# xuhao1/TaichiSLAM

Hardware: AMD Instinct MI355X
Metric: depth-frames/s integrated (640x480->512^3 TSDF) (higher is better)
Workload: dtype f16 storage / f32 + int64 fixed-point arithmetic; 1 GPU; BASELINE configs[1]: single 640x480 u16 depth stream (sphere room r=3 m, 1 deg/frame) -> DenseTSDF 512^3 / 2 cm, recast_step 2, max_ray 5 m; one stream+submap per GPU

## Files before the change

### taichislam_amd/csrc/tsl_integrate.hip

```cpp
#include "tsl_tsdf.hpp"
#include <hip/hip_ext.h>

namespace tsl {

#ifdef TSL_TIMING
#define TSL_T0() const int _wv = (blockIdx.x * (int)blockDim.x + (int)threadIdx.x) >> 6
#define TSL_TICK(F, k) do { long long _n = wall_clock64(); if (lane_id() == 0 && _wv < 16384) (F).dbg[_wv * 16 + (k)] = _n; } while (0)
#else
#define TSL_T0() do {} while (0)
#define TSL_TICK(F, k) do {} while (0)
#endif

#define SCATTER_TILE 4096

struct RayRegs { float pf0, pf1, pf2, d0, d1, d2, P0, P1, P2, w; long long qden; int n; };

__device__ __forceinline__ uint32_t wave_min_u32(uint32_t v)
{
    for (int d = 32; d > 0; d >>= 1) { const uint32_t o = (uint32_t)__shfl_xor((int)v, d); v = o < v ? o : v; }
    return v;
}
__device__ __forceinline__ RayRegs make_ray(const uint4 rec, int n, const FrameParams& P)
{
    RayRegs R;
// ... 553 lines not shown
{
    if (all_small) {
#pragma unroll
        for (int q = 0; q < N; ++q) nv[q] = apply_update_f(old[q], from_fix32(qn[q]), from_fix32(qd[q]));
    } else {
#pragma unroll
        for (int q = 0; q < N; ++q) nv[q] = apply_update_f(old[q], from_fix(qn[q]), from_fix(qd[q]));
    }
}

__device__ __forceinline__ int uni(int v) { return __builtin_amdgcn_readfirstlane(v); }
#define IT_UNIT 0
#define IT_POOL 1
#define IT_SLAB 2
#define IT_NP   3
#define IT_TMALL 4
#define IT_FMASK 5
#define IT_OFF  6
#define IT_N    (IT_OFF + TSL_NB)
#define IT_WORDS (IT_N + TSL_NB + 2)
#define NRANGE (PLAN_NCLS * (TSL_NB + 1))

template <bool TEX, bool FASTDIV, int NT, int SPT, int WPE>
__global__ void __launch_bounds__(NT, WPE) k_integrate_batch(MapDev M, BatchDev B, int kind)
{
    constexpr int CSEGS = SPT * NT, VPT = TSL_BRK3 / NT, CH = VPT < FLUSH_CHUNK ? VPT : FLUSH_CHUNK;
    static_assert(VPT <= 16, "the written / first-touch masks hold 16 voxels per thread");
#ifdef TSL_EXP_SLOT16
    __shared__ ulonglong2 s_acc[TSL_BRK3];
#define S_NUM(i) s_acc[i].x
#define S_DEN(i) s_acc[i].y
#else
    __shared__ unsigned long long s_num[TSL_BRK3];
    __shared__ unsigned long long s_den[TSL_BRK3];
#define S_NUM(i) s_num[i]
#define S_DEN(i) s_den[i]
#endif
    __shared__ unsigned long long s_keys[CSEGS];
    __shared__ uint32_t s_win[TEX ? TSL_BRK3 : 1];
    __shared__ int s_bin[64];
    __shared__ int s_claim[2];
    __shared__ int s_uq[TSL_NB];
    __shared__ int s_cum[NRANGE + 1];
    __shared__ int s_it[3][IT_WORDS];
    uint32_t okmask = 0u;
#pragma unroll
    for (int q = 0; q < TSL_NB; ++q) if (q < B.n) {
        const FrameDev& Fq = B.f[q];
        if (Fq.counters[HDR_FAIL] == 0) okmask |= 1u << q;
        const int nact = min(Fq.counters[1], Fq.max_frame_bricks);
        for (int i = blockIdx.x * NT + threadIdx.x; i < nact; i += gridDim.x * NT) { const int b = Fq.act_b[i]; Fq.bhist[b] = 0; Fq.bcursor[b] = 0; }
    }
    if (threadIdx.x < TSL_NB) s_uq[threadIdx.x] = 0;
    if (threadIdx.x == 0) {
        int acc = 0, k = 0;
#ifdef TSL_CLASS_MAJOR
        for (int c = 0; c < PLAN_NCLS; ++c) {
            s_cum[k++] = acc; acc += min(B.f[0].counters[HDR_UNITS + c], B.f[0].unit_cap);
            for (int q = 0; q < TSL_NB; ++q) { s_cum[k++] = acc; if ((okmask >> q) & 1u) acc += min(B.f[q].counters[HDR_PARTS + c], B.f[q].part_cap); }
        }
#else
        for (int c = 0; c < PLAN_NCLS; ++c) { s_cum[k++] = acc; if (kind != 2) acc += min(B.f[0].counters[HDR_UNITS + c], B.f[0].unit_cap); }
        for (int c = 0; c < PLAN_NCLS; ++c)
            for (int q = 0; q < TSL_NB; ++q) { s_cum[k++] = acc; if (kind != 1 && ((okmask >> q) & 1u)) acc += min(B.f[q].counters[HDR_PARTS + c], B.f[q].part_cap); }
#endif
        s_cum[NRANGE] = acc;
        s_claim[0] = __hip_atomic_fetch_add(&B.f[0].counters[kind == 2 ? HDR_CLAIM2 : HDR_CLAIM], 1, __ATOMIC_RELAXED, __HIP_MEMORY_SCOPE_AGENT);
    }
    __syncthreads();
    const int total = uni(s_cum[NRANGE]);
    int* const claim = &B.f[0].counters[kind == 2 ? HDR_CLAIM2 : HDR_CLAIM];
    auto entry_of = [&](int r, int* kq) -> int4 {
        int k = 0;
#pragma unroll
        for (int j = 1; j < NRANGE; ++j) k += r >= uni(s_cum[j]) ? 1 : 0;
#ifdef TSL_CLASS_MAJOR
// ... 23 lines not shown
            int pool = e.z;
            if (fm == 0u) { fm = 1u; pool = -1; }
            it[IT_UNIT] = kq < 0 ? 1 : 0; it[IT_POOL] = pool; it[IT_SLAB] = kq < 0 ? 0 : e.w; it[IT_NP] = kq < 0 ? 1 : (e.y >> 16) & ((1 << PART_NP_BITS) - 1);
            it[IT_TMALL] = (int)tm; it[IT_FMASK] = (int)fm;
        }
    };
    const int r0 = uni(s_claim[0]);
    if (r0 >= total) return;
    { int kq, io, in; const int4 e = entry_of(r0, &kq); info_of(e, kq, &io, &in); commit(0, e, kq, io, in); }
    __syncthreads();
    auto steps_of = [&](int sl, uint32_t fm) -> int {
        int n = 0;
#pragma unroll
        for (int q = 0; q < TSL_NB; ++q) if ((fm >> q) & 1u) n += max(1, (uni(s_it[sl][IT_N + q]) + CSEGS - 1) / CSEGS);
        return n;
    };
    long long uniq = 0;
    int t = 0, slot = 0, c = 0; (void)t;
    int n_known = 0;
    bool exhausted = false;
    int f = __builtin_ctz((uint32_t)uni(s_it[0][IT_FMASK]));

    unsigned long long kk[SPT]; uint4 recs[SPT]; uint32_t wids[SPT];
#define TSL_SORT_DEAL(KIN, NSEG, FD)                                                                                    \
    {                                                                                                                   \
        int rr[SPT];                                                                                                    \
        _Pragma("unroll") for (int q = 0; q < SPT; ++q) {                                                               \
            const int i = q * NT + (int)threadIdx.x; rr[q] = -1;                                                        \
            if (i < (NSEG)) rr[q] = atomicAdd(&s_bin[63 - (int)(KIN[q] & 63ull)], 1);                                   \
        }                                                                                                               \
        __syncthreads();                                                                                                \
        if (threadIdx.x < 64) {                                                                                         \
            const int cb = s_bin[threadIdx.x]; int inc = cb;                                                            \
            for (int d = 1; d < 64; d <<= 1) { const int o = __shfl_up(inc, d); if ((int)threadIdx.x >= d) inc += o; }  \
            s_bin[threadIdx.x] = inc - cb;                                                                              \
        }                                                                                                               \
        __syncthreads();                                                                                                \
        _Pragma("unroll") for (int q = 0; q < SPT; ++q) if (rr[q] >= 0) s_keys[s_bin[63 - (int)(KIN[q] & 63ull)] + rr[q]] = KIN[q]; \
        __syncthreads();                                                                                                \
        _Pragma("unroll") for (int q = 0; q < SPT; ++q) {                                                               \
            const int i = q * NT + ((q & 1) ? NT - 1 - (int)threadIdx.x : (int)threadIdx.x);                            \
            if (i < (NSEG)) {                                                                                           \
                kk[q] = s_keys[i];                                                                                      \
                const int r = (int)((kk[q] >> (SEG_CNT_BITS + SEG_J_BITS)) & ((1u << STG_RAY_BITS) - 1));               \
                recs[q] = (FD).rayA[r];                                                                                 \
                wids[q] = TEX ? (FD).rayFirst[r] + 1u : 0u;                                                             \
            }                                                                                                           \
        }                                                                                                               \
        if (threadIdx.x < 64) s_bin[threadIdx.x] = 0;               \
    }
#define TSL_PRIME(SL, FQ)                                                                                               \
    {                                                                                                                   \
        const FrameDev& F0 = B.f[FQ];                                                                                   \
        const int off0 = uni(s_it[SL][IT_OFF + (FQ)]), nseg0 = min(uni(s_it[SL][IT_N + (FQ)]), CSEGS);                  \
        unsigned long long k0[SPT];                                                                                     \
        _Pragma("unroll") for (int q = 0; q < SPT; ++q) { const int i = q * NT + threadIdx.x; k0[q] = i < nseg0 ? F0.seg_sorted[off0 + i] : 0ull; } \
        TSL_SORT_DEAL(k0, nseg0, F0)                                                                                    \
    }

    {
#ifdef TSL_EXP_SLOT16
        for (int i = threadIdx.x; i < TSL_BRK3; i += NT) s_acc[i] = make_ulonglong2(0ull, 0ull);
#else
        ulonglong2* zn = reinterpret_cast<ulonglong2*>(s_num); ulonglong2* zd = reinterpret_cast<ulonglong2*>(s_den);
        for (int i = threadIdx.x; i < TSL_BRK3 / 2; i += NT) { zn[i] = make_ulonglong2(0ull, 0ull); zd[i] = make_ulonglong2(0ull, 0ull); }
#endif
        if (TEX) for (int i = threadIdx.x; i < TSL_BRK3; i += NT) s_win[i] = 0u;
        if (threadIdx.x < 64) s_bin[threadIdx.x] = 0;
        __syncthreads();
        TSL_PRIME(0, f)
    }
    uint32_t old[VPT];
// ... 30 lines not shown
        const bool has_next = !last_step || n_known >= 1;
        int fx = f, cx = c + 1, slotx = slot;
        if (last_chunk) {
            cx = 0;
            if (!last_frame) fx = f + 1 + __builtin_ctz(later);
            else if (has_next) { slotx = slot1; fx = __builtin_ctz((uint32_t)uni(s_it[slotx][IT_FMASK])); }
        }
        const FrameDev& Fx = B.f[fx];
        unsigned long long kn[SPT];
        const int offx = uni(s_it[slotx][IT_OFF + fx]) + cx * CSEGS;
        const int nsegn = has_next ? min(CSEGS, uni(s_it[slotx][IT_N + fx]) - cx * CSEGS) : 0;
#pragma unroll
        for (int q = 0; q < SPT; ++q) { const int i = q * NT + threadIdx.x; kn[q] = i < nsegn ? Fx.seg_sorted[offx + i] : 0ull; }
        const uint32_t* const twr = M.tw + (size_t)(p >= 0 ? p : 0) * TSL_BRK3;
        if (first_step) { have_old = false; vmask = 0u; }
        if (!TEX && unit && p >= 0 && first_step) {
#pragma unroll
            for (int q = 0; q < VPT; ++q) old[q] = twr[q * NT + threadIdx.x];
            have_old = true;
        }
#pragma unroll
        for (int q = 0; q < SPT; ++q) {
            const int i = q * NT + ((q & 1) ? NT - 1 - (int)threadIdx.x : (int)threadIdx.x);
            if (i >= nseg) continue;
            const unsigned long long key = kk[q];
            const int cnt = (int)(key & ((1u << SEG_CNT_BITS) - 1)), j0 = (int)((key >> SEG_CNT_BITS) & ((1u << SEG_J_BITS) - 1));
            const RayRegs R = make_ray(recs[q], 0, P);
            const uint32_t wid = wids[q];
#ifndef TSL_EXP_STAGGER
#define TSL_EXP_STAGGER 27
#endif
            int off = ((int)((threadIdx.x * (unsigned)TSL_EXP_STAGGER) & 63u) * cnt) >> 6;
            for (int s = 0; s < cnt; s += 2) {
                const int ja = j0 + off; off = (off + 1 == cnt) ? 0 : off + 1;
                const int jb = j0 + off; off = (off + 1 == cnt) ? 0 : off + 1;
                int la, lb; float qa, qb;
                step_eval<FASTDIV>(R, K, ja, &la, &qa);
                step_eval<FASTDIV>(R, K, jb, &lb, &qb);
                long long na = (long long)(int)qa, nb = (long long)(int)qb;
                if (__builtin_expect(__any(!(fabsf(qa) < 2147483648.0f) || !(fabsf(qb) < 2147483648.0f)), 0)) { na = __float2ll_rn(qa); nb = __float2ll_rn(qb); }
                atomicAdd(&S_NUM(la), (unsigned long long)na);
                atomicAdd(&S_DEN(la), (unsigned long long)R.qden);
                if (TEX) atomicMax(&s_win[la], wid);
                const bool vb = s + 1 < cnt;
#ifdef TSL_EXP_ADDZERO
                atomicAdd(&S_NUM(lb), (unsigned long long)(vb ? nb : 0ll));
                atomicAdd(&S_DEN(lb), (unsigned long long)(vb ? R.qden : 0ll));
// ... 93 lines not shown
        const long long _td = wall_clock64();
#endif
        {
            const long long u = wave_sum_ll(uniq);
            if (lane_id() == 0 && u) atomicAdd(&s_uq[f], (int)u);
            uniq = 0;
        }
        if (fetching) { commit(n_known == 0 ? slot1 : slot2, ne, nkq, nio, nin); ++n_known; }
#ifdef TSL_TIMING
        if (threadIdx.x == 0 && last_step) _rec[4] = wall_clock64();
        if (threadIdx.x == 0) { _ph[2] += _td - _tc; _ph[3] += wall_clock64() - _td; }
#endif
        if (!has_next && n_known == 0) break;
        __syncthreads();
        c = 0;
        if (last_frame) { ++t; slot = slot1; --n_known; f = __builtin_ctz((uint32_t)uni(s_it[slot][IT_FMASK])); }
        else f = fx;
        if (!has_next) TSL_PRIME(slot, f)
    }
#undef TSL_PRIME
#undef TSL_SORT_DEAL
    __syncthreads();
    if (threadIdx.x < TSL_NB && s_uq[threadIdx.x]) atomic_add_i64(&B.f[threadIdx.x].stats->unique, (long long)s_uq[threadIdx.x]);
}

#ifndef APPLY_SPLIT
#define APPLY_SPLIT 8
#endif
#ifndef APPLY_ROUND
#define APPLY_ROUND 2
#endif
template <bool TEX>
__global__ void __launch_bounds__(256) k_apply_slab(MapDev M, BatchDev B)
{
    __shared__ int s_uq[TSL_NB];
    constexpr int VP = TSL_BRK3 / APPLY_SPLIT / 256;
    uint32_t okmask = 0u;
#pragma unroll
    for (int q = 0; q < TSL_NB; ++q) if (q < B.n && B.f[q].counters[HDR_FAIL] == 0) okmask |= 1u << q;
    const int nheavy = min(B.f[0].counters[HDR_HEAVY], B.f[0].max_frame_bricks);
    const ulonglong2* const slab = reinterpret_cast<const ulonglong2*>(B.f[0].acc);
    if (threadIdx.x < TSL_NB) s_uq[threadIdx.x] = 0;
    __syncthreads();
    for (int item = blockIdx.x; item < nheavy * APPLY_SPLIT; item += gridDim.x) {
        const int4 e = B.f[0].heavy_tab[item / APPLY_SPLIT];
        const int b = e.x, p = e.y;
// ... 83 lines not shown
int launch_segments(tsl_tsdf* m, const BatchDev& B, const FrameParams* hp, int total, hipStream_t st)
{
    const FrameParams& P = hp[0];
    if (P.variant != 2) return TSL_OK;
    const int iblocks = (int)(((int64_t)total * P.split + 255) / 256);
    prof_begin(m, TSL_K_SEGMENTS, st);
    if (P.group) hipLaunchKernelGGL(k_segments<true>, dim3(iblocks, B.n), dim3(256), 0, st, m->M, B);
    else hipLaunchKernelGGL(k_segments<false>, dim3(iblocks, B.n), dim3(256), 0, st, m->M, B);
    prof_end(m, st);
    int unit_max = m->unit_max <= m->unit_floor ? m->unit_max : std::max(m->unit_floor, (int)((long long)m->unit_max * B.n / TSL_NB));
    int unit_half = std::min(unit_max, m->unit_half <= 2048 ? m->unit_half : std::max(2048, (int)((long long)m->unit_half * B.n / TSL_NB)));
    if (P.seq && m->seq_impl) unit_max = unit_half = 1 << 30;
    prof_begin(m, TSL_K_BIN, st);
    hipLaunchKernelGGL(k_plan, dim3((B.f[0].max_frame_bricks + 255) / 256, B.n), dim3(256), 0, st, m->M, B, m->chunks * m->wg * m->spt, unit_max, unit_half);
    hipLaunchKernelGGL(k_scatter, dim3(256, B.n), dim3(256), 0, st, B);
    prof_end(m, st);
    return TSL_OK;
}

int launch_brick(tsl_tsdf* m, const BatchDev& B, const FrameParams& P, int kind, hipStream_t st, hipEvent_t start, hipEvent_t stop)
{
    const int bg = kind == 2 ? m->pgrid : (B.n <= 2 ? (m->bgrid + 1) / 2 : (kind == 1 ? m->ugrid : m->bgrid));
#define TSL_LAUNCH_IB(TEXV, FD) do { \
        if (m->wg == 512 && m->spt == 2 && !TEXV) hipExtLaunchKernelGGL((k_integrate_batch<false, FD, 512, 2, 4>), dim3((2 * m->ncu * bg + 99) / 100), dim3(512), 0, st, start, stop, 0, m->M, B, kind); \
        else if (m->wg == 512) hipExtLaunchKernelGGL((k_integrate_batch<TEXV, FD, 512, 4, 2>), dim3((m->ncu * bg + 99) / 100), dim3(512), 0, st, start, stop, 0, m->M, B, kind); \
        else hipExtLaunchKernelGGL((k_integrate_batch<TEXV, FD, 256, 4, (TEXV ? 1 : 2)>), dim3(((TEXV ? 1 : 2) * m->ncu * bg + 99) / 100), dim3(256), 0, st, start, stop, 0, m->M, B, kind); } while (0)
    if (P.tex) { if (P.fastdiv) TSL_LAUNCH_IB(true, true); else TSL_LAUNCH_IB(true, false); }
    else { if (P.fastdiv) TSL_LAUNCH_IB(false, true); else TSL_LAUNCH_IB(false, false); }
#undef TSL_LAUNCH_IB
    TSL_HIP(hipGetLastError());
    return TSL_OK;
}
int launch_slab_apply(tsl_tsdf* m, const BatchDev& B, const FrameParams& P)
{
    prof_begin(m, TSL_K_FINALIZE);
    if (P.tex) hipLaunchKernelGGL(k_apply_slab<true>, dim3(16 * m->ncu), dim3(256), 0, m->stream_, m->M, B);
    else hipLaunchKernelGGL(k_apply_slab<false>, dim3(16 * m->ncu), dim3(256), 0, m->stream_, m->M, B);
    prof_end(m);
    TSL_HIP(hipGetLastError());
    return TSL_OK;
}
int launch_apply_batch(tsl_tsdf* m, const BatchDev& B, const FrameParams& P, hipEvent_t start, hipEvent_t stop)
{
    const int rc = launch_brick(m, B, P, 0, m->stream_, start, stop);
    return rc ? rc : launch_slab_apply(m, B, P);
}

int launch_apply(tsl_tsdf* m, FSet& S, int total)
{
// ... 16 lines not shown
```

### taichislam_amd/csrc/tsl_tsdf.hip

```cpp
#include "tsl_tsdf.hpp"
#include <rocprim/rocprim.hpp>
#include <algorithm>
#include <cmath>
#include <cstdio>
#include <cstdlib>
#include <cstring>
#include <mutex>

namespace tsl {

static thread_local std::string g_err;
void set_error(const std::string& s) { g_err = s; }

__device__ __forceinline__ uint32_t part1by2_32(uint32_t x)
{
    x &= 0x3ffu;
    x = (x ^ (x << 16)) & 0xff0000ffu;
    x = (x ^ (x << 8)) & 0x0300f00fu;
    x = (x ^ (x << 4)) & 0x030c30c3u;
    x = (x ^ (x << 2)) & 0x09249249u;
    return x;
}
__device__ __forceinline__ uint64_t part1by2_64(uint64_t x)
{
// ... 318 lines not shown
        uint32_t* ob = reinterpret_cast<uint32_t*>(M.obs + (size_t)p * TSL_BRK3);
        uint32_t* oc = reinterpret_cast<uint32_t*>(M.occ + (size_t)p * TSL_BRK3);
        for (int l = threadIdx.x; l < TSL_BRK3; l += 256) tw[l] = 0u;
        for (int l = threadIdx.x; l < TSL_BRK3 / 4; l += 256) { ob[l] = 0u; oc[l] = 0u; }
        if (M.col) { uint2* c = reinterpret_cast<uint2*>(M.col + (size_t)p * TSL_BRK3 * 4); for (int l = threadIdx.x; l < TSL_BRK3; l += 256) c[l] = make_uint2(0u, 0u); }
        if (threadIdx.x == 0) M.table[M.owner[p]] = TSL_EMPTY;
    }
}

__global__ void __launch_bounds__(256) k_verify_div(float vs, float rvs, unsigned long long* bad)
{
    unsigned long long nbad = 0;
    for (unsigned long long i = (unsigned long long)blockIdx.x * 256 + threadIdx.x; i < (1ull << 32); i += (unsigned long long)gridDim.x * 256) {
        const float x = __uint_as_float((uint32_t)i);
        const float ax = fabsf(x);
        if (!(ax >= 7.8886090522101181e-31f) || !(ax < 2147483648.0f * vs)) continue;
        const float q = x / vs;
        const float f = div_vs(x, vs, rvs, 1);
        if (__float_as_uint(q) != __float_as_uint(f)) ++nbad;
    }
    if (nbad) atomicAdd(bad, nbad);
}

__global__ void __launch_bounds__(256) k_selftest(int which, unsigned long long* bad)
{
    unsigned long long nbad = 0;
    for (unsigned long long i = (unsigned long long)blockIdx.x * 256 + threadIdx.x; i < (1ull << 32); i += (unsigned long long)gridDim.x * 256) {
        const float x = __uint_as_float((uint32_t)i);
        if (which == 0) {
            if (!(fabsf(x) < 2147483648.0f)) continue;
            if (rnd_i(x) != rnd_i_ref(x)) ++nbad;
        } else {
            if (!(x >= 1.2621774483536189e-29f) || !(x < INFINITY)) continue;
            if (__float_as_uint(sqrt_rn_norm(x)) != __float_as_uint(sqrt_rn(x))) ++nbad;
        }
    }
    if (nbad) atomicAdd(bad, nbad);
}

int grow(void** p, size_t* have, size_t need)
{
    if (*have >= need) return TSL_OK;
    if (*p) (void)hipFree(*p);
    *p = nullptr; *have = 0;
    size_t want = need + need / 4 + 4096;
    TSL_HIP(hipMalloc(p, want));
    *have = want;
    return TSL_OK;
}
// ... 417 lines not shown
                                      (size_t)m->F.max_points, 0u, 64u, m->stream_));
    *bytes = a > b ? a : b;
    return TSL_OK;
}

static void fill_frame_params(tsl_tsdf* m, const double R[9], const double T[3])
{
    const int s = m->active;
    convert_pose(&m->baseR[(size_t)s * 9], &m->baseT[(size_t)s * 3], R, T, m->P.R, m->P.T);
    m->P.slot = map_slot(m, s);
    m->P.variant = m->variant; m->P.split = (m->variant == 2 && m->split > 8) ? 8 : m->split;
}

}

using namespace tsl;

extern "C" {

const char* tsl_version(void) { return "taichislam_hip 0.1 (gfx950)"; }
const char* tsl_last_error(void) { return g_err.c_str(); }
int tsl_selftest(int which, int64_t* mismatches)
{
    TSL_REQUIRE(mismatches && which >= 0 && which <= 2, "tsl_selftest: bad argument");
    unsigned long long* bad = nullptr;
    TSL_HIP(hipMalloc((void**)&bad, sizeof(unsigned long long)));
    TSL_HIP(hipMemset(bad, 0, sizeof(unsigned long long)));
    if (which == 2) (void)selftest_seqdiv(bad);
    else hipLaunchKernelGGL(k_selftest, dim3(8192), dim3(256), 0, 0, which, bad);
    unsigned long long h = ~0ull;
    hipError_t e = hipMemcpy(&h, bad, sizeof(h), hipMemcpyDeviceToHost);
    (void)hipFree(bad);
    TSL_HIP(e);
    *mismatches = (int64_t)h;
    return TSL_OK;
}
int tsl_device_count(int* n)
{
    int c = 0;
    hipError_t e = hipGetDeviceCount(&c);
    if (e != hipSuccess) { c = 0; }
    if (n) *n = c;
    return TSL_OK;
}

static int init_handle(tsl_tsdf* m, const tsl_tsdf_cfg* cfg, int device)
{
    m->cfg = *cfg; m->device = device; m->bytes = 0;
    (void)hipGetLastError();
    TSL_HIP(hipStreamCreateWithFlags(&m->stream_, hipStreamNonBlocking));
    m->overlap = TSL_NB; m->last_set = 0;
    for (auto& S : m->fset) { S.sort_temp = nullptr; S.header = nullptr; S.Pd = nullptr; S.stage_in = nullptr; S.stage_in_bytes = 0; S.stage_tex = nullptr; S.stage_tex_bytes = 0; S.pin = nullptr; S.pin_bytes = 0; S.pin_dev = nullptr; S.copy_in = S.copy_tex = S.copy_tex_off = 0; }
// ... 21 lines not shown
    FrameParams& P = m->P; std::memset(&P, 0, sizeof(P));
    for (int i = 0; i < 3; ++i) P.R[i * 4] = 1.0f;
    P.vs = (float)cfg->voxel_scale;
    {
        const float y0 = (float)(1.0 / (double)P.vs);
        float best = y0; double err = std::fabs(1.0 - (double)y0 * (double)P.vs);
        const float cand[2] = { std::nextafterf(y0, 0.0f), std::nextafterf(y0, INFINITY) };
        for (float c : cand) { const double e = std::fabs(1.0 - (double)c * (double)P.vs); if (e < err) { err = e; best = c; } }
        P.rvs = best; P.fastdiv = 0;
    }
    P.thr_max = (float)(cfg->max_ray_length * 1000.0); P.thr_min = (float)(cfg->min_ray_length * 1000.0);
    P.max_ray_f = (float)cfg->max_ray_length;
    P.max_steps_f = (float)(cfg->max_ray_length / cfg->voxel_scale);
    P.internal_f = (float)cfg->internal_voxels;
    P.pcl_lo = m->pcl_lo; P.pcl_ext = m->pcl_ext; P.pcl_bits = m->pcl_bits; P.pcl_blk = blk; P.seq = 0;
    P.step = cfg->recast_step; P.same_proj = cfg->color_same_proj;
    m->surf_thres = (float)(cfg->voxel_scale * 1.8);
    m->disp_floor = (float)cfg->disp_floor; m->disp_ceiling = (float)cfg->disp_ceiling;
    m->baseR.assign((size_t)m->npose * 9, 0.0); m->baseT.assign((size_t)m->npose * 3, 0.0);
    m->baseRf.assign((size_t)m->npose * 9, 0.0f); m->baseTf.assign((size_t)m->npose * 3, 0.0f);
    for (int s = 0; s < m->npose; ++s) for (int i = 0; i < 3; ++i) { m->baseR[(size_t)s * 9 + i * 4] = 1.0; m->baseRf[(size_t)s * 9 + i * 4] = 1.0f; }
    std::memset(m->gbaseR, 0, sizeof(m->gbaseR)); std::memset(m->gbaseT, 0, sizeof(m->gbaseT));
    for (int i = 0; i < 3; ++i) m->gbaseR[i * 4] = 1.0;
    m->P.group = 1; m->phases = 3; m->wg = 512; m->spt = 2; m->adaptive = 0; m->ramp_batches = 2; m->ramp_size = 4; m->bgrid = 75; m->ugrid = 75; m->pgrid = 25; m->split_launch = 0; m->chunks = 4; m->unit_max = 1024 * TSL_NB; m->unit_half = 1 << 20; m->unit_floor = 4096; m->batch_gen = 0;
    { hipDeviceProp_t pr; TSL_HIP(hipGetDeviceProperties(&pr, device)); m->ncu = pr.multiProcessorCount > 0 ? pr.multiProcessorCount : 256; }
    m->active = 0; m->variant = 2; m->split = 2; m->semantics = 0; m->seq_impl = 1; m->seq_ready = false; m->seq_bytes0 = 0; m->seq_d = nullptr; m->seq_tuple_cap = 0;
    m->prof_on = false; m->prof_open = false; m->prof_group = false; m->prof_mask = ~0u; std::memset(m->prof_ms, 0, sizeof(m->prof_ms)); std::memset(m->prof_n, 0, sizeof(m->prof_n));
    m->sort_temp = nullptr; m->sort_temp_bytes = 0;
    m->xbuf = nullptr; m->xbuf_bytes = 0; m->mesh_v = m->mesh_n = m->mesh_c = nullptr; m->mesh_count = nullptr; m->mesh_cap = 0; m->mesh_flags = nullptr;
    m->fuse_acc = nullptr; m->fuse_cnt = nullptr; m->fuse_cacc = nullptr; m->fuse_dirty = false; m->mrg_nunion = -1;
    m->esdf = nullptr; m->esdf_par = nullptr; m->esdf_ok = nullptr; m->esdf_mode = 0; m->esdf_grid = 0; m->fuse_direct = false; m->merge_exchange = 0; m->mrg_racc = m->mrg_rcnt = m->mrg_rec = nullptr; m->mrg_racc_bytes = m->mrg_rcnt_bytes = m->mrg_rec_bytes = 0; m->esdf_orphans = 0; m->esdf_last = nullptr; m->esdf_in = nullptr; m->esdf_read = nullptr; m->esdf_overlap = true; m->esdf_ctr_idx = 0; for (int k = 0; k < 2; ++k) { m->fseq_keys[k] = m->fseq_vals[k] = nullptr; m->fseq_bytes[k] = m->fseq_vbytes[k] = 0; } m->fseq_temp = nullptr; m->fseq_tbytes = 0; m->fseq_ctr = nullptr; m->esdf_gate = nullptr; m->esdf_gate_ev = nullptr; m->esdf_gate_set = false; m->esdf_gate_mask = 0; m->esdf_valid = false; m->esdf_force_full = false; m->pose_dev = nullptr;

    MapDev& M = m->M; std::memset(&M, 0, sizeof(M));
    M.N = m->N; M.Nz = m->Nz; M.nbx = m->nbx; M.nbz = m->nbz; M.nb3 = m->nb3; M.nsub = m->nsub; M.hN = m->N / 2; M.hNz = m->Nz / 2;
    int64_t want = cfg->max_bricks > 0 ? cfg->max_bricks : 32768 * (int64_t)(m->nsub > 4 ? 4 : (m->nsub > 1 ? m->nsub : 1));
    const int64_t all = (int64_t)m->nsub * m->nb3;
    if (want > all) want = all;
    M.max_bricks = (int)want;
    int rc;
    if ((rc = dev_alloc(m, (void**)&M.table, sizeof(int) * (size_t)all, 0xff))) return rc;
    if ((rc = dev_alloc(m, (void**)&M.tw, sizeof(uint32_t) * (size_t)want * TSL_BRK3, 0))) return rc;
    if ((rc = dev_alloc(m, (void**)&M.obs, (size_t)want * TSL_BRK3, 0))) return rc;
    if ((rc = dev_alloc(m, (void**)&M.occ, (size_t)want * TSL_BRK3, 0))) return rc;
    if (cfg->texture_enabled) { if ((rc = dev_alloc(m, (void**)&M.col, sizeof(uint16_t) * 4 * (size_t)want * TSL_BRK3, 0))) return rc; }
    if ((rc = dev_alloc(m, (void**)&M.owner, sizeof(int) * (size_t)want, 0))) return rc;
    if ((rc = dev_alloc(m, (void**)&M.touch, (size_t)want, 0))) return rc;
    if ((rc = dev_alloc(m, (void**)&M.pool_top, sizeof(int) * 4, 0))) return rc;
// ... 145 lines not shown
{
    TSL_HIP(hipMemcpyAsync(m->h_ints, dev, sizeof(int), hipMemcpyDeviceToHost, ms(m)));
    TSL_HIP(hipStreamSynchronize(ms(m)));
    *out = m->h_ints[0];
    return take_deferred(m);
}
static int check_dev_err(tsl_tsdf* m) { (void)ms(m); return take_dev_err(m); }
int tsl_tsdf_get_option(tsl_tsdf* m, const char* name, int* value)
{
    TSL_REQUIRE(m && name && value, "null");
    if (!std::strcmp(name, "group")) { *value = m->P.group; return TSL_OK; }
    if (!std::strcmp(name, "esdf_mode")) { *value = m->esdf_mode; return TSL_OK; }
    if (!std::strcmp(name, "fuse_window_misses")) { return read_int(m, m->M.pool_top + 2, value); }
    if (!std::strcmp(name, "esdf_orphans")) { int rc = esdf_finish(m); if (rc) return rc; *value = (int)m->esdf_orphans; return TSL_OK; }
    if (!std::strcmp(name, "semantics")) { *value = m->semantics; return TSL_OK; }
    if (!std::strcmp(name, "seq_impl")) { *value = m->seq_impl; return TSL_OK; }
    if (!std::strcmp(name, "last_heavy_bricks") || !std::strcmp(name, "last_slab_slots")) {
        TSL_REQUIRE(m->scratch_ready, "nothing integrated yet");
        int rc = tsl_tsdf_sync(m); if (rc) return rc;
        const int bi = (m->cur + TSL_NBATCH - 1) % TSL_NBATCH;
        int v[40];
        TSL_HIP(hipMemcpy(v, m->fset[bi * TSL_NB].F.counters, sizeof(v), hipMemcpyDeviceToHost));
        *value = name[5] == 'h' ? v[14] : v[13];
        return TSL_OK;
    }
    if (!std::strcmp(name, "seq_longest_run")) {
        TSL_REQUIRE(m->scratch_ready, "nothing integrated yet");
        int rc = tsl_tsdf_sync(m); if (rc) return rc;
        const int bi = (m->cur + TSL_NBATCH - 1) % TSL_NBATCH;
        long long sum = 0;
        for (int q = 0; q < m->last_batch_n; ++q) { int v[40]; TSL_HIP(hipMemcpy(v, m->fset[bi * TSL_NB + q].F.counters, sizeof(v), hipMemcpyDeviceToHost)); sum += (unsigned)v[31]; }
        *value = (int)(sum > 0x7fffffffll ? 0x7fffffffll : sum);
        return TSL_OK;
    }
    if (!std::strcmp(name, "seq_long_voxels")) {
        TSL_REQUIRE(m->scratch_ready, "nothing integrated yet");
        int rc = tsl_tsdf_sync(m); if (rc) return rc;
        const int bi = (m->cur + TSL_NBATCH - 1) % TSL_NBATCH;
        int v[40]; TSL_HIP(hipMemcpy(v, m->fset[bi * TSL_NB].F.counters, sizeof(v), hipMemcpyDeviceToHost));
        *value = v[28] + v[30];
#ifdef TSL_SEQ_DBG
        fprintf(stderr, "seq dbg (long role, last batch): evaluations %d, commits that moved T %d, commits that moved W only %d\n", v[32], v[33], v[34]);
#endif
        return TSL_OK;
    }
    if (!std::strcmp(name, "fastdiv")) { *value = m->P.fastdiv; return TSL_OK; }
// ... 387 lines not shown
                if (seq_prepare(m)) m->semantics = 0;
                return rc;
            }
        }
        return TSL_OK;
    }
    if (!std::strcmp(name, "fastdiv")) { if (value == 0) m->P.fastdiv = 0; return TSL_OK; }
    if (!std::strcmp(name, "mesh_gather")) { m->mesh_gather = value != 0; return TSL_OK; }
    if (!std::strcmp(name, "esdf_full")) { m->esdf_force_full = value != 0; return TSL_OK; }
    if (!std::strcmp(name, "esdf_mode")) { TSL_REQUIRE(value == 0 || value == 1, "esdf_mode: 0 = regional recompute (default), 1 = raise / lower wavefront with parent directions"); int rc = esdf_finish(m); if (rc) return rc; m->esdf_mode = value; m->esdf_valid = false; return TSL_OK; }
    if (!std::strcmp(name, "esdf_round_cap")) { m->esdf_round_cap = value; return TSL_OK; }
    if (!std::strcmp(name, "merge_exchange")) { TSL_REQUIRE(value == 0 || value == 1, "merge_exchange: 0 = all-reduce of the packed sums, 1 = reduce-scatter + all-gather of finalised voxels"); m->merge_exchange = value; return TSL_OK; }
    if (!std::strcmp(name, "fuse_direct")) { m->fuse_direct = value != 0; return TSL_OK; }
    if (!std::strcmp(name, "esdf_grid")) { TSL_REQUIRE(value >= 0, "esdf_grid: workgroups of a relaxation round (0 = four per CU)"); m->esdf_grid = value; return TSL_OK; }
    if (!std::strcmp(name, "esdf_overlap")) { int rc = esdf_finish(m); if (rc) return rc; m->esdf_overlap = value != 0; return TSL_OK; }
    if (!std::strcmp(name, "unit")) { TSL_REQUIRE(value >= 0 && value <= (1 << 20), "unit must be 0..2^20 segments"); int rc = tsl_tsdf_sync(m); if (rc) return rc; m->unit_max = value; return TSL_OK; }
    if (!std::strcmp(name, "unit_floor")) { TSL_REQUIRE(value >= 0 && value <= (1 << 20), "unit_floor must be 0..2^20 segments"); int rc = tsl_tsdf_sync(m); if (rc) return rc; m->unit_floor = value; return TSL_OK; }
    if (!std::strcmp(name, "unit_half")) { TSL_REQUIRE(value >= 0 && value <= (1 << 20), "unit_half must be 0..2^20 segments"); int rc = tsl_tsdf_sync(m); if (rc) return rc; m->unit_half = value; return TSL_OK; }
    if (!std::strcmp(name, "chunks")) { TSL_REQUIRE(value >= 1 && value <= 8, "chunks must be 1..8"); int rc = tsl_tsdf_sync(m); if (rc) return rc; m->chunks = value; return TSL_OK; }
    if (!std::strcmp(name, "adaptive")) { m->adaptive = value != 0; return TSL_OK; }
    if (!std::strcmp(name, "ramp_size")) { TSL_REQUIRE(value >= 1 && value <= TSL_NB, "ramp_size must be 1..8 frames"); m->ramp_size = value; return TSL_OK; }
    if (!std::strcmp(name, "ramp")) { TSL_REQUIRE(value >= 0 && value <= 16, "ramp must be 0..16 half batches"); m->ramp_batches = value; return TSL_OK; }
    if (!std::strcmp(name, "ugrid") || !std::strcmp(name, "pgrid")) { TSL_REQUIRE(value >= 5 && value <= 200, "ugrid / pgrid must be 5..200 (percent of the resident workgroup slots)"); { int rc = tsl_tsdf_sync(m); if (rc) return rc; } (name[0] == 'u' ? m->ugrid : m->pgrid) = value; return TSL_OK; }
    if (!std::strcmp(name, "split_launch")) { TSL_REQUIRE(value == 0 || value == 1, "split_launch must be 0 or 1"); { int rc = tsl_tsdf_sync(m); if (rc) return rc; } m->split_launch = value; return TSL_OK; }
    if (!std::strcmp(name, "bgrid")) { TSL_REQUIRE(value >= 10 && value <= 200, "bgrid must be 10..200 (percent of the resident workgroup slots)"); { int rc = tsl_tsdf_sync(m); if (rc) return rc; } m->bgrid = value; return TSL_OK; }
    if (!std::strcmp(name, "spt")) { TSL_REQUIRE(value == 2 || value == 4, "spt must be 2 or 4"); { int rc = tsl_tsdf_sync(m); if (rc) return rc; } m->spt = value; return TSL_OK; }
    if (!std::strcmp(name, "wg")) { TSL_REQUIRE(value == 256 || value == 512, "wg must be 256 or 512"); { int rc = tsl_tsdf_sync(m); if (rc) return rc; } m->wg = value; return TSL_OK; }
    if (!std::strcmp(name, "phases")) { int rc = tsl_tsdf_sync(m); if (rc) return rc; m->phases = value & 3; return TSL_OK; }
    if (!std::strcmp(name, "overlap")) { int rc = tsl_tsdf_sync(m); if (rc) return rc; m->overlap = value < 0 ? 0 : (value > TSL_NB ? TSL_NB : value); for (auto& H : m->batch) H.b_pending = false; return TSL_OK; }
    if (!std::strcmp(name, "split")) { TSL_REQUIRE(value >= 1 && value <= 64 && (64 % value) == 0, "split must divide 64"); m->split = value; return TSL_OK; }
    set_error("unknown option"); return TSL_ERR_ARG;
}

}
```

### taichislam_amd/csrc/tsl_tsdf.hpp

```cpp
#pragma once
#include "tsl_common.hpp"

namespace tsl {

struct FrameParams {
    float R[9], T[3];
    float fx, fy, cx, cy;
    float fxc, fyc, cxc, cyc;
    float vs;
    float rvs; int fastdiv;
    float thr_max, thr_min;
    float max_ray_f;
    float max_steps_f;
    float internal_f;
    int   pcl_lo, pcl_ext, pcl_bits;
    int   step, hh, ww, H, W;
    int   rstride;
    int   cstride;
    int   th, tw, tex, same_proj;
    int   slot;
    int   variant, split;
    int   group;
    int   seq, pcl_blk;
    int   hlog2;
// ... 35 lines not shown
#define SEG_CNT_BITS 6
#define SEG_J_BITS   12
#define SEG_RAY_BITS 24
#define SEG_SLOT_SHIFT (SEG_CNT_BITS + SEG_J_BITS + SEG_RAY_BITS)
#define SEG_MAX_CNT 63
#define STG_RAY_BITS 22
#define STG_B_SHIFT (SEG_CNT_BITS + SEG_J_BITS + STG_RAY_BITS)
#define PART_NP_BITS 12
#define SLAB_SLOT_BITS 20
#define PLAN_NCLS 4
#define HDR_FAIL 11
#define HDR_CLAIM 12
#define HDR_SLAB 13
#define HDR_HEAVY 14
#define HDR_PARTS 16
#define HDR_UNITS 20
#define HDR_CLAIM2 24
#define HDR_SEQ_TUPLES 26
#define HDR_SEQ_LONG 28
#define HDR_SEQ_XLONG 30
#define HDR_SEQ_MAXRUN 31
#define HDR_SEQ_CLAIM 35
#define HDR_SEQ_SLOTS 29

__device__ __forceinline__ void frame_fail(const MapDev& M, const FrameDev& F, int bits) { atomicOr(&F.counters[11], bits); atomicOr(M.err, bits); }

#define H_INL 13
#define H_BLOCK_SHIFT 44
#define H_EMPTY 0ull
__device__ __forceinline__ unsigned long long h_key(unsigned long long vkey, int block) { return (vkey | ((unsigned long long)block << H_BLOCK_SHIFT)) + 1ull; }
#define GROUP_BIG_CAP 16384
struct HSlot { unsigned long long key; int cnt; uint32_t pix[H_INL]; };
static_assert(sizeof(HSlot) == 64, "one slot per 64 bytes");
__device__ __forceinline__ uint32_t h_hash64(unsigned long long key, int log2n) { return (uint32_t)((key * 0x9E3779B97F4A7C15ull) >> (64 - log2n)); }

struct PixAcc { int cnt; h16 sx, sy, sz, zs, cr, cg, cb; };

__device__ __forceinline__ void acc_colour(const FrameParams& P, const FrameDev& F, uint32_t pid, PixAcc& A)
{
    const uint8_t* rgb;
    if (P.points) rgb = P.tex_input + (size_t)pid * 3;
    else {
        const int jj = (int)pid / P.ww, ii = (int)pid - jj * P.ww;
        const int pj = jj * P.step, pi = ii * P.step;
        if (P.same_proj) rgb = P.tex_input + ((size_t)pj * P.tw + pi) * 3;
        else {
// ... 118 lines not shown
    uint32_t* mesh_flags;
    float *mesh_v, *mesh_n, *mesh_c; int* mesh_count; int64_t mesh_cap; int mesh_gather;
    void *fuse_acc, *fuse_cnt, *fuse_cacc; bool fuse_dirty;
    uint8_t* mrg_mask; int *mrg_list, *mrg_count; int mrg_nunion;
    void *mrg_pacc, *mrg_pcnt; size_t mrg_pacc_bytes, mrg_pcnt_bytes;
    void *mrg_racc, *mrg_rcnt, *mrg_rec; size_t mrg_racc_bytes, mrg_rcnt_bytes, mrg_rec_bytes; int merge_exchange;
    float* esdf; uint8_t *esdf_fl, *esdf_region, *esdf_par, *esdf_ok; int esdf_mode, esdf_grid; bool fuse_direct; long long esdf_orphans; int *esdf_list, *esdf_queue, *esdf_ctr, *esdf_inq, *esdf_nbr; uint32_t* esdf_note; int esdf_qcap;
    float *esdf_exp_xyz, *esdf_exp_val; int* esdf_exp_count; int esdf_exp_n;
    bool esdf_valid, esdf_force_full; int esdf_submap; float esdf_gamma, esdf_maxd; tsl_esdf_stats esdf_stats;
    bool esdf_query_ok; int* esdf_q_ctr; int esdf_q_rounds;
    hipEvent_t esdf_gate, esdf_gate_ev; bool esdf_gate_set; unsigned esdf_gate_mask;
    hipEvent_t esdf_in, esdf_read, esdf_last;
    bool esdf_overlap; int esdf_ctr_idx;
    void *fseq_keys[2], *fseq_vals[2], *fseq_temp; size_t fseq_bytes[2], fseq_vbytes[2], fseq_tbytes; void* fseq_ctr;
    EsdfSlot esdf_slot[TSL_ESDF_SLOTS]; int esdf_tail, esdf_npend, esdf_rounds_seen, esdf_round_cap; bool esdf_short; tsl_esdf_totals_t esdf_tot;
    bool prof_on, prof_open, prof_group; unsigned prof_mask; std::vector<tsl::ProfSlot> prof; std::vector<hipEvent_t> prof_free;
    double prof_ms[TSL_K_COUNT]; int64_t prof_n[TSL_K_COUNT];
    int semantics;
    int seq_impl;
    bool seq_ready; int64_t seq_bytes0;
    tsl::SeqDev seq_h[TSL_NSETS]; tsl::SeqDev* seq_d;
    void *seqb_keys[TSL_NBATCH][2], *seqb_vals[TSL_NBATCH][2], *seqb_temp[TSL_NBATCH], *seqb_long[TSL_NBATCH], *seqb_lmask[TSL_NBATCH], *seqb_perm[TSL_NBATCH]; size_t seqb_temp_bytes; long long seq_tuple_cap;
    unsigned long long *seq_keys[2], *seq_vals[2], *seq_ctr; void* seq_temp; size_t seq_temp_bytes; long long seq_cap;
    int variant, split, phases, wg, spt, ncu, chunks, unit_max, unit_half, unit_floor, bgrid, ugrid, pgrid, split_launch, adaptive, ramp, ramp_batches, ramp_size; bool clean; uint64_t batch_gen;
    int64_t bytes;
    void* seqv_sum[TSL_NBATCH]; int* seqv_log;
    uint32_t shape_hash; int dry_launches;
};

namespace tsl {
int  grow(void** p, size_t* have, size_t need);
hipStream_t ms(tsl_tsdf* m);
int  flush_pending(tsl_tsdf* m);
void prof_begin(tsl_tsdf* m, int kid, hipStream_t st = nullptr, int count = 1);
void prof_end(tsl_tsdf* m, hipStream_t st = nullptr);
bool prof_slot(tsl_tsdf* m, int kid, int count, hipEvent_t* a, hipEvent_t* b);
void convert_pose(const double* Rb, const double* Tb, const double* R, const double* T, float* outR, float* outT);
int  dev_alloc(tsl_tsdf* m, void** p, size_t bytes, int fill);
int  check_variant2(tsl_tsdf* m);
int  launch_segments(tsl_tsdf* m, const BatchDev& B, const FrameParams* hp, int total, hipStream_t st);
int  launch_apply(tsl_tsdf* m, FSet& S, int total);
int  launch_apply_batch(tsl_tsdf* m, const BatchDev& B, const FrameParams& P, hipEvent_t start = nullptr, hipEvent_t stop = nullptr);
int  launch_brick(tsl_tsdf* m, const BatchDev& B, const FrameParams& P, int kind, hipStream_t st, hipEvent_t start, hipEvent_t stop);
int  launch_slab_apply(tsl_tsdf* m, const BatchDev& B, const FrameParams& P);
int  launch_seq_group(tsl_tsdf* m, const BatchDev& B, const FrameParams* hp, int bi, hipStream_t st);
int  launch_seq_apply(tsl_tsdf* m, const BatchDev& B, const FrameParams& P, int bi);
void seq_release(tsl_tsdf* m);
// ... 8 lines not shown
```

Measured before the change: 34530 frames/s.

## Split ray segments into pieces across idle threads in light integrate steps

When a step in the batched integrate kernel has few segments relative to the workgroup's segment capacity, each segment is dealt out in up to 2^seg_split pieces with even-length voxel counts, so more threads share the per-ray march work. This targets underutilised workgroups on light steps. The cost is extra key decoding, redundant ray-record loads per piece, and per-block counter atomics for split statistics. A selftest and a tunable knob (default max split) are added.

```diff
diff --git a/taichislam_amd/csrc/tsl_integrate.hip b/taichislam_amd/csrc/tsl_integrate.hip
--- a/taichislam_amd/csrc/tsl_integrate.hip
+++ b/taichislam_amd/csrc/tsl_integrate.hip
@@ -599,8 +599,9 @@
 #define NRANGE (PLAN_NCLS * (TSL_NB + 1))
 
 template <bool TEX, bool FASTDIV, int NT, int SPT, int WPE>
-__global__ void __launch_bounds__(NT, WPE) k_integrate_batch(MapDev M, BatchDev B, int kind)
-{
+__global__ void __launch_bounds__(NT, WPE) k_integrate_batch(MapDev M, BatchDev B, int kind_cap)
+{
+    const int kind = kind_cap & 3, split_cap = kind_cap >> 2;
     constexpr int CSEGS = SPT * NT, VPT = TSL_BRK3 / NT, CH = VPT < FLUSH_CHUNK ? VPT : FLUSH_CHUNK;
     static_assert(VPT <= 16, "the written / first-touch masks hold 16 voxels per thread");
 #ifdef TSL_EXP_SLOT16
@@ -618,6 +619,7 @@
     __shared__ int s_bin[64];
     __shared__ int s_claim[2];
     __shared__ int s_uq[TSL_NB];
+    __shared__ int s_split[SEG_SPLIT_MAX + 1];
     __shared__ int s_cum[NRANGE + 1];
     __shared__ int s_it[3][IT_WORDS];
     uint32_t okmask = 0u;
@@ -629,6 +631,7 @@
         for (int i = blockIdx.x * NT + threadIdx.x; i < nact; i += gridDim.x * NT) { const int b = Fq.act_b[i]; Fq.bhist[b] = 0; Fq.bcursor[b] = 0; }
     }
     if (threadIdx.x < TSL_NB) s_uq[threadIdx.x] = 0;
+    if (threadIdx.x <= SEG_SPLIT_MAX) s_split[threadIdx.x] = 0;
     if (threadIdx.x == 0) {
         int acc = 0, k = 0;
 #ifdef TSL_CLASS_MAJOR
@@ -698,6 +701,7 @@
     int f = __builtin_ctz((uint32_t)uni(s_it[0][IT_FMASK]));
 
     unsigned long long kk[SPT]; uint4 recs[SPT]; uint32_t wids[SPT];
+    int wsh = 0;
 #define TSL_SORT_DEAL(KIN, NSEG, FD)                                                                                    \
     {                                                                                                                   \
         int rr[SPT];                                                                                                    \
@@ -714,16 +718,20 @@
         __syncthreads();                                                                                                \
         _Pragma("unroll") for (int q = 0; q < SPT; ++q) if (rr[q] >= 0) s_keys[s_bin[63 - (int)(KIN[q] & 63ull)] + rr[q]] = KIN[q]; \
         __syncthreads();                                                                                                \
+        const int sh_ = seg_split_shift((NSEG), CSEGS, split_cap);                                                      \
         _Pragma("unroll") for (int q = 0; q < SPT; ++q) {                                                               \
             const int i = q * NT + ((q & 1) ? NT - 1 - (int)threadIdx.x : (int)threadIdx.x);                            \
-            if (i < (NSEG)) {                                                                                           \
-                kk[q] = s_keys[i];                                                                                      \
+            if (i < ((NSEG) << sh_)) {                                                                                  \
+                kk[q] = s_keys[i >> sh_];                                                                               \
+                if (sh_) kk[q] = seg_piece(kk[q], sh_, i & ((1 << sh_) - 1));        \
                 const int r = (int)((kk[q] >> (SEG_CNT_BITS + SEG_J_BITS)) & ((1u << STG_RAY_BITS) - 1));               \
                 recs[q] = (FD).rayA[r];                                                                                 \
                 wids[q] = TEX ? (FD).rayFirst[r] + 1u : 0u;                                                             \
             }                                                                                                           \
         }                                                                                                               \
         if (threadIdx.x < 64) s_bin[threadIdx.x] = 0;               \
+        if (threadIdx.x == 0 && (NSEG) > 0) atomicAdd(&s_split[sh_], 1);    \
+        wsh = sh_;                                                                                                      \
     }
 #define TSL_PRIME(SL, FQ)                                                                                               \
     {                                                                                                                   \
@@ -800,7 +808,7 @@
 #pragma unroll
         for (int q = 0; q < SPT; ++q) {
             const int i = q * NT + ((q & 1) ? NT - 1 - (int)threadIdx.x : (int)threadIdx.x);
-            if (i >= nseg) continue;
+            if (i >= (nseg << wsh)) continue;
             const unsigned long long key = kk[q];
             const int cnt = (int)(key & ((1u << SEG_CNT_BITS) - 1)), j0 = (int)((key >> SEG_CNT_BITS) & ((1u << SEG_J_BITS) - 1));
             const RayRegs R = make_ray(recs[q], 0, P);
@@ -940,6 +948,7 @@
 #undef TSL_SORT_DEAL
     __syncthreads();
     if (threadIdx.x < TSL_NB && s_uq[threadIdx.x]) atomic_add_i64(&B.f[threadIdx.x].stats->unique, (long long)s_uq[threadIdx.x]);
+    if (threadIdx.x <= SEG_SPLIT_MAX && s_split[threadIdx.x]) atomicAdd(&B.f[0].counters[HDR_SPLIT + threadIdx.x], s_split[threadIdx.x]);
 }
 
 #ifndef APPLY_SPLIT
@@ -1069,9 +1078,9 @@
 {
     const int bg = kind == 2 ? m->pgrid : (B.n <= 2 ? (m->bgrid + 1) / 2 : (kind == 1 ? m->ugrid : m->bgrid));
 #define TSL_LAUNCH_IB(TEXV, FD) do { \
-        if (m->wg == 512 && m->spt == 2 && !TEXV) hipExtLaunchKernelGGL((k_integrate_batch<false, FD, 512, 2, 4>), dim3((2 * m->ncu * bg + 99) / 100), dim3(512), 0, st, start, stop, 0, m->M, B, kind); \
-        else if (m->wg == 512) hipExtLaunchKernelGGL((k_integrate_batch<TEXV, FD, 512, 4, 2>), dim3((m->ncu * bg + 99) / 100), dim3(512), 0, st, start, stop, 0, m->M, B, kind); \
-        else hipExtLaunchKernelGGL((k_integrate_batch<TEXV, FD, 256, 4, (TEXV ? 1 : 2)>), dim3(((TEXV ? 1 : 2) * m->ncu * bg + 99) / 100), dim3(256), 0, st, start, stop, 0, m->M, B, kind); } while (0)
+        if (m->wg == 512 && m->spt == 2 && !TEXV) hipExtLaunchKernelGGL((k_integrate_batch<false, FD, 512, 2, 4>), dim3((2 * m->ncu * bg + 99) / 100), dim3(512), 0, st, start, stop, 0, m->M, B, kind | (m->seg_split << 2)); \
+        else if (m->wg == 512) hipExtLaunchKernelGGL((k_integrate_batch<TEXV, FD, 512, 4, 2>), dim3((m->ncu * bg + 99) / 100), dim3(512), 0, st, start, stop, 0, m->M, B, kind | (m->seg_split << 2)); \
+        else hipExtLaunchKernelGGL((k_integrate_batch<TEXV, FD, 256, 4, (TEXV ? 1 : 2)>), dim3(((TEXV ? 1 : 2) * m->ncu * bg + 99) / 100), dim3(256), 0, st, start, stop, 0, m->M, B, kind | (m->seg_split << 2)); } while (0)
     if (P.tex) { if (P.fastdiv) TSL_LAUNCH_IB(true, true); else TSL_LAUNCH_IB(true, false); }
     else { if (P.fastdiv) TSL_LAUNCH_IB(false, true); else TSL_LAUNCH_IB(false, false); }
 #undef TSL_LAUNCH_IB
diff --git a/taichislam_amd/csrc/tsl_tsdf.hip b/taichislam_amd/csrc/tsl_tsdf.hip
--- a/taichislam_amd/csrc/tsl_tsdf.hip
+++ b/taichislam_amd/csrc/tsl_tsdf.hip
@@ -364,9 +364,47 @@
     if (nbad) atomicAdd(bad, nbad);
 }
 
+__device__ int selftest_split_case(int i)
+{
+    if (i < 64 * 3 * 4) {
+        const int cnt = i & 63, sh = (i >> 6) & 3, jsel = i >> 8;
+        const int j0 = jsel == 0 ? 0 : (jsel == 1 ? 1 : 4032);
+        int nbad = 0;
+        for (int pat = 0; pat < 2; ++pat) {
+            const unsigned long long hi = (pat ? 0xa5c3961e5a3c69e1ull : ~0ull) << (SEG_CNT_BITS + SEG_J_BITS);
+            const unsigned long long key = hi | ((unsigned long long)j0 << SEG_CNT_BITS) | (unsigned long long)cnt;
+            const int len = ((cnt + (2 << sh) - 1) >> (sh + 1)) << 1;
+            unsigned long long seen = 0ull; bool ok = (len & 1) == 0;
+            for (int u = 0; u < (1 << sh); ++u) {
+                const unsigned long long pk = seg_piece(key, sh, u);
+                const int c = (int)(pk & 63ull), j = (int)((pk >> SEG_CNT_BITS) & 4095ull);
+                ok = ok && (pk >> (SEG_CNT_BITS + SEG_J_BITS)) == (key >> (SEG_CNT_BITS + SEG_J_BITS)) && c <= len;
+                for (int s = 0; s < c; ++s) {
+                    const int r = j + s - j0;
+                    if (r < 0 || r >= cnt || ((seen >> r) & 1ull)) ok = false; else seen |= 1ull << r;
+                }
+            }
+            ok = ok && seen == (1ull << cnt) - 1ull;
+            nbad += ok ? 0 : 1;
+        }
+        return nbad;
+    }
+    i -= 64 * 3 * 4;
+    const int nseg = i % 2049, csegs = ((i / 2049) & 1) ? 2048 : 1024, cap = i / (2049 * 2);
+    const int sh = seg_split_shift(nseg, csegs, cap);
+    if (sh < 0 || sh > cap) return 1;
+    if (nseg > csegs) return sh == 0 ? 0 : 1;
+    if ((nseg << sh) > csegs) return 1;
+    return sh == cap || (nseg << (sh + 1)) > csegs ? 0 : 1;
+}
 __global__ void __launch_bounds__(256) k_selftest(int which, unsigned long long* bad)
 {
     unsigned long long nbad = 0;
+    if (which == 3) {
+        for (int i = blockIdx.x * 256 + threadIdx.x; i < 64 * 3 * 4 + 2049 * 2 * (SEG_SPLIT_MAX + 1); i += gridDim.x * 256) nbad += selftest_split_case(i);
+        if (nbad) atomicAdd(bad, nbad);
+        return;
+    }
     for (unsigned long long i = (unsigned long long)blockIdx.x * 256 + threadIdx.x; i < (1ull << 32); i += (unsigned long long)gridDim.x * 256) {
         const float x = __uint_as_float((uint32_t)i);
         if (which == 0) {
@@ -830,12 +868,12 @@
 const char* tsl_last_error(void) { return g_err.c_str(); }
 int tsl_selftest(int which, int64_t* mismatches)
 {
-    TSL_REQUIRE(mismatches && which >= 0 && which <= 2, "tsl_selftest: bad argument");
+    TSL_REQUIRE(mismatches && which >= 0 && which <= 3, "tsl_selftest: bad argument");
     unsigned long long* bad = nullptr;
     TSL_HIP(hipMalloc((void**)&bad, sizeof(unsigned long long)));
     TSL_HIP(hipMemset(bad, 0, sizeof(unsigned long long)));
     if (which == 2) (void)selftest_seqdiv(bad);
-    else hipLaunchKernelGGL(k_selftest, dim3(8192), dim3(256), 0, 0, which, bad);
+    else hipLaunchKernelGGL(k_selftest, dim3(which == 3 ? 128 : 8192), dim3(256), 0, 0, which, bad);
     unsigned long long h = ~0ull;
     hipError_t e = hipMemcpy(&h, bad, sizeof(h), hipMemcpyDeviceToHost);
     (void)hipFree(bad);
@@ -903,7 +941,7 @@
     for (int s = 0; s < m->npose; ++s) for (int i = 0; i < 3; ++i) { m->baseR[(size_t)s * 9 + i * 4] = 1.0; m->baseRf[(size_t)s * 9 + i * 4] = 1.0f; }
     std::memset(m->gbaseR, 0, sizeof(m->gbaseR)); std::memset(m->gbaseT, 0, sizeof(m->gbaseT));
     for (int i = 0; i < 3; ++i) m->gbaseR[i * 4] = 1.0;
-    m->P.group = 1; m->phases = 3; m->wg = 512; m->spt = 2; m->adaptive = 0; m->ramp_batches = 2; m->ramp_size = 4; m->bgrid = 75; m->ugrid = 75; m->pgrid = 25; m->split_launch = 0; m->chunks = 4; m->unit_max = 1024 * TSL_NB; m->unit_half = 1 << 20; m->unit_floor = 4096; m->batch_gen = 0;
+    m->P.group = 1; m->phases = 3; m->wg = 512; m->spt = 2; m->adaptive = 0; m->ramp_batches = 2; m->ramp_size = 4; m->bgrid = 75; m->ugrid = 75; m->pgrid = 25; m->split_launch = 0; m->seg_split = SEG_SPLIT_MAX; m->chunks = 4; m->unit_max = 1024 * TSL_NB; m->unit_half = 1 << 20; m->unit_floor = 4096; m->batch_gen = 0;
     { hipDeviceProp_t pr; TSL_HIP(hipGetDeviceProperties(&pr, device)); m->ncu = pr.multiProcessorCount > 0 ? pr.multiProcessorCount : 256; }
     m->active = 0; m->variant = 2; m->split = 2; m->semantics = 0; m->seq_impl = 1; m->seq_ready = false; m->seq_bytes0 = 0; m->seq_d = nullptr; m->seq_tuple_cap = 0;
     m->prof_on = false; m->prof_open = false; m->prof_group = false; m->prof_mask = ~0u; std::memset(m->prof_ms, 0, sizeof(m->prof_ms)); std::memset(m->prof_n, 0, sizeof(m->prof_n));
@@ -1095,6 +1133,16 @@
         int v[40];
         TSL_HIP(hipMemcpy(v, m->fset[bi * TSL_NB].F.counters, sizeof(v), hipMemcpyDeviceToHost));
         *value = name[5] == 'h' ? v[14] : v[13];
+        return TSL_OK;
+    }
+    if (!std::strcmp(name, "seg_split")) { *value = m->seg_split; return TSL_OK; }
+    if (!std::strncmp(name, "last_split_steps", 16) && name[16] >= '0' && name[16] <= '0' + SEG_SPLIT_MAX && !name[17]) {
+        TSL_REQUIRE(m->scratch_ready, "nothing integrated yet");
+        int rc = tsl_tsdf_sync(m); if (rc) return rc;
+        const int bi = (m->cur + TSL_NBATCH - 1) % TSL_NBATCH;
+        int v[40];
+        TSL_HIP(hipMemcpy(v, m->fset[bi * TSL_NB].F.counters, sizeof(v), hipMemcpyDeviceToHost));
+        *value = v[HDR_SPLIT + (name[16] - '0')];
         return TSL_OK;
     }
     if (!std::strcmp(name, "seq_longest_run")) {
@@ -1528,6 +1576,7 @@
     if (!std::strcmp(name, "ramp_size")) { TSL_REQUIRE(value >= 1 && value <= TSL_NB, "ramp_size must be 1..8 frames"); m->ramp_size = value; return TSL_OK; }
     if (!std::strcmp(name, "ramp")) { TSL_REQUIRE(value >= 0 && value <= 16, "ramp must be 0..16 half batches"); m->ramp_batches = value; return TSL_OK; }
     if (!std::strcmp(name, "ugrid") || !std::strcmp(name, "pgrid")) { TSL_REQUIRE(value >= 5 && value <= 200, "ugrid / pgrid must be 5..200 (percent of the resident workgroup slots)"); { int rc = tsl_tsdf_sync(m); if (rc) return rc; } (name[0] == 'u' ? m->ugrid : m->pgrid) = value; return TSL_OK; }
+    if (!std::strcmp(name, "seg_split")) { TSL_REQUIRE(value >= 0 && value <= SEG_SPLIT_MAX, "seg_split must be 0..3 (a light step deals a segment out in up to 2^seg_split pieces)"); { int rc = tsl_tsdf_sync(m); if (rc) return rc; } m->seg_split = value; return TSL_OK; }
     if (!std::strcmp(name, "split_launch")) { TSL_REQUIRE(value == 0 || value == 1, "split_launch must be 0 or 1"); { int rc = tsl_tsdf_sync(m); if (rc) return rc; } m->split_launch = value; return TSL_OK; }
     if (!std::strcmp(name, "bgrid")) { TSL_REQUIRE(value >= 10 && value <= 200, "bgrid must be 10..200 (percent of the resident workgroup slots)"); { int rc = tsl_tsdf_sync(m); if (rc) return rc; } m->bgrid = value; return TSL_OK; }
     if (!std::strcmp(name, "spt")) { TSL_REQUIRE(value == 2 || value == 4, "spt must be 2 or 4"); { int rc = tsl_tsdf_sync(m); if (rc) return rc; } m->spt = value; return TSL_OK; }
diff --git a/taichislam_amd/csrc/tsl_tsdf.hpp b/taichislam_amd/csrc/tsl_tsdf.hpp
--- a/taichislam_amd/csrc/tsl_tsdf.hpp
+++ b/taichislam_amd/csrc/tsl_tsdf.hpp
@@ -81,6 +81,25 @@
 #define HDR_SEQ_MAXRUN 31
 #define HDR_SEQ_CLAIM 35
 #define HDR_SEQ_SLOTS 29
+#define HDR_SPLIT 36
+
+#define SEG_SPLIT_MAX 3
+__host__ __device__ __forceinline__ int seg_split_shift(int nseg, int csegs, int cap)
+{
+    int sh = 0;
+    while (sh < cap && (nseg << (sh + 1)) <= csegs) ++sh;
+    return sh;
+}
+__host__ __device__ __forceinline__ unsigned long long seg_piece(unsigned long long key, int sh, int u)
+{
+    const uint32_t lo = (uint32_t)key, fields = (1u << (SEG_CNT_BITS + SEG_J_BITS)) - 1u;
+    const int cnt = (int)(lo & ((1u << SEG_CNT_BITS) - 1u)), j0 = (int)((lo >> SEG_CNT_BITS) & ((1u << SEG_J_BITS) - 1u));
+    const int len = ((cnt + (2 << sh) - 1) >> (sh + 1)) << 1;
+    const int o = u * len, left = cnt - o;
+    const int c = left < 0 ? 0 : (left < len ? left : len);
+    const uint32_t nlo = (lo & ~fields) | ((uint32_t)(c > 0 ? j0 + o : j0) << SEG_CNT_BITS) | (uint32_t)c;
+    return (key & 0xffffffff00000000ull) | nlo;
+}
 
 __device__ __forceinline__ void frame_fail(const MapDev& M, const FrameDev& F, int bits) { atomicOr(&F.counters[11], bits); atomicOr(M.err, bits); }
 
@@ -245,7 +264,7 @@
     tsl::SeqDev seq_h[TSL_NSETS]; tsl::SeqDev* seq_d;
     void *seqb_keys[TSL_NBATCH][2], *seqb_vals[TSL_NBATCH][2], *seqb_temp[TSL_NBATCH], *seqb_long[TSL_NBATCH], *seqb_lmask[TSL_NBATCH], *seqb_perm[TSL_NBATCH]; size_t seqb_temp_bytes; long long seq_tuple_cap;
     unsigned long long *seq_keys[2], *seq_vals[2], *seq_ctr; void* seq_temp; size_t seq_temp_bytes; long long seq_cap;
-    int variant, split, phases, wg, spt, ncu, chunks, unit_max, unit_half, unit_floor, bgrid, ugrid, pgrid, split_launch, adaptive, ramp, ramp_batches, ramp_size; bool clean; uint64_t batch_gen;
+    int variant, split, phases, wg, spt, ncu, chunks, unit_max, unit_half, unit_floor, bgrid, ugrid, pgrid, split_launch, seg_split, adaptive, ramp, ramp_batches, ramp_size; bool clean; uint64_t batch_gen;
     int64_t bytes;
     void* seqv_sum[TSL_NBATCH]; int* seqv_log;
     uint32_t shape_hash; int dry_launches;
```

Result: slower. 34120 frames/s (-1.2%).
